# limitz/cuda-audio

Measured on AMD Instinct MI355X. Metric: real-time factor (frames/s / 44.1k), stereo block=256, 10 s IR, higher is better.
Workload: dtype f32

## Files before the change

cuda_audio_amd/csrc/mcconv.hip:

```cpp
#include <hip/hip_runtime.h>
#include <immintrin.h>

#include <algorithm>
#include <atomic>
#include <chrono>
#include <cmath>
#include <cstdarg>
#include <cstdio>
#include <cstdlib>
#include <cstring>
#include <mutex>
#include <new>
#include <vector>

#include "../../include/mcconv.h"
#include "params_handoff.h"
#include "kernels.hip.h"
#include "ossave.hip.h"
#include "singlefft.hip.h"
#include "resample.hip.h"
#include "irshape.hip.h"
#include "ireq.hip.h"
#include "irdecay.hip.h"

// ... 1104 lines not shown
            if (pe[nv] <= pb[nv]) continue;
            list[nv] = act[a];
            if (per_slot_gains) list[nv].uniform = false;
            nv++;
        }
        mo->nsum = std::max(1, nv) * kNchunk;
        if (!nv) HIP_TRY(hipMemsetAsync(e->d_part, 0, sizeof(float4) * (size_t)T * MC_NB * mo->nsum, e->stream));
        for (int a = 0; a < nv; a++) {
            launch_mac_stream(e, list[a], pb[a], pe[a], T, slot0, mo->nsum, a * kNchunk);
            mo->swept = std::max(mo->swept, pe[a] - pb[a]);
        }
        mo->ysrc = e->d_part;
        mo->sk = mo->nsum;
        mo->stt = (int64_t)MC_NB * mo->nsum;
    }
    return MC_OK;
}

Retired make_retired(const mc_engine* e) {
    Retired r;
    r.mac = e->d_res_mac;
    r.fix = e->d_res_fix;
    r.rr = e->rr;
    r.end = (int64_t)e->res_end;
    r.b0 = (int64_t)e->epoch_b0;
    return r;
}

int zero_ring_range(mc_engine* e, float* ring, uint64_t from, uint64_t to) {
    if (to <= from) return MC_OK;
    const uint64_t rr = (uint64_t)e->rr;
    const uint64_t a = from & (rr - 1), n = to - from;
    const uint64_t n1 = std::min(n, rr - a);
    for (int c = 0; c < 2; c++) {
        HIP_TRY(hipMemsetAsync(ring + (size_t)c * rr + a, 0, sizeof(float) * n1, e->stream));
        if (n > n1) HIP_TRY(hipMemsetAsync(ring + (size_t)c * rr, 0, sizeof(float) * (n - n1), e->stream));
    }
    return MC_OK;
}

int retire_epoch(mc_engine* e, uint64_t new_delay, bool force = false) {
    if (new_delay == e->cur_delay && !force) return MC_OK;
    if (e->t_front == e->epoch_b0) {
        e->cur_delay = new_delay;
        return MC_OK;
    }
    if (e->pipe_count) return fail(MC_ERR_STATE, "predelay change / voice merge while a batch awaits mc_finish_batch_device");
    if (e->sliced) return fail(MC_ERR_STATE, "predelay change / voice merge on a block-sliced engine (mc_reset first)");
    {
        int rc = drain_post(e);
        if (!rc) rc = leave_jack_path(e);
        if (rc) return rc;
    }
    const uint64_t b0 = e->t_front, bs = e->epoch_b0, d_old = e->cur_delay;
    const uint64_t new_end = (b0 - (uint64_t)e->pm) * MC_B + e->cfg.n_ref;
    const uint64_t pending_from = std::max<uint64_t>(e->res_end, b0 * MC_B);
    int rc = zero_ring_range(e, e->d_res_mac, pending_from, new_end);
    if (!rc) rc = zero_ring_range(e, e->d_res_fix, pending_from, new_end);
    if (rc) return rc;

    ActiveVoice act[MC_MAXV];
    int vir[2][MC_MAXV];
    const int nact = collect_voices(e, nullptr, act, vir, nullptr);
    int F = 0;
    for (int a = 0; a < nact; a++) F = std::max(F, act[a].p_end);
    F = (int)std::min<uint64_t>((uint64_t)F, (new_end - b0 * MC_B + MC_B - 1) / MC_B);
    if (d_old)
        hipLaunchKernelGGL(k_flush_ring, dim3((unsigned)((d_old + 255) / 256)), dim3(256), 0, e->stream, e->d_wet, e->wr,
                           (int64_t)(b0 * MC_B), (int64_t)d_old, e->d_res_mac, e->rr, (int64_t)new_end);
    uint64_t tv = b0;
    while (F > 0) {
        int Tc = std::min(F, e->Tcap);
        if (!(Tc >= e->stream_threshold && !e->half)) Tc = std::min(Tc, e->Tstream);
        const int slot0 = (int)(tv & (uint64_t)(e->ring - 1));
        hipLaunchKernelGGL(k_fwd<false>, dim3((Tc + FWD_TILE - 1) / FWD_TILE), dim3(XF_THREADS), 0, e->stream, (const float*)nullptr,
                           (const float*)nullptr, 1, (int64_t)0, Tc, e->d_fdl, e->ring, slot0, (const BlockParams*)nullptr, 0,
                           (float4*)nullptr, (float4*)nullptr, e->d_tw, e->d_fdl16, (float*)nullptr, 0, (float4*)nullptr, 0,
                           (int64_t)0, 0, Tc, Tc, 0, 0, DropAhead(), 0);
        MacOut mo;
        rc = launch_mac_batch(e, act, nact, true, Tc, slot0, &mo);
        if (rc) return rc;
        launch_inv(e, mo, tv, e->stream);
        hipLaunchKernelGGL(k_flush_ola, dim3(Tc), dim3(256), 0, e->stream, e->d_seg, e->sr, (int64_t)tv, (int64_t)d_old,
                           e->d_res_mac, e->rr, (int64_t)new_end);
        tv += (uint64_t)Tc;
        F -= Tc;
    }
    {
        const uint64_t n = new_end - b0 * MC_B;
        hipLaunchKernelGGL(k_flush_fix, dim3((unsigned)((n + MC_B - 1) / MC_B)), dim3(256), 0, e->stream, e->d_cring, e->rc,
                           e->d_res_fix, e->rr, (int64_t)(b0 * MC_B), (int64_t)new_end, (int64_t)bs, (int64_t)b0 - 1, (int64_t)d_old,
                           (int64_t)e->cfg.n_ref, (int)e->cfg.compat, make_taildrop(e, vir, d_old), e->pm);
    }
    HIP_TRY(hipGetLastError());
    HIP_TRY(hipMemsetAsync(e->d_fdl, 0, sizeof(float4) * (size_t)MC_NB * e->ring, e->stream));
    if (e->d_fdl16) HIP_TRY(hipMemsetAsync(e->d_fdl16, 0, sizeof(uint2) * (size_t)MC_NB * e->ring, e->stream));
    HIP_TRY(hipMemsetAsync(e->d_seg, 0, sizeof(float) * (size_t)e->sr * 2 * FFT_N, e->stream));
    HIP_TRY(hipMemsetAsync(e->d_wet, 0, sizeof(float) * 2 * (size_t)e->wr, e->stream));
    e->res_end = new_end;
    e->epoch_b0 = b0;
    e->cur_delay = new_delay;
    e->spec_valid = e->dspec.valid = false;
    return MC_OK;
}

void corr_chunks(CorrArgs* ca, int T, int need_a0, int need_a1, int need_b0) {
    ca->need_a0 = need_a0;
    ca->need_a1 = need_a1;
    ca->need_b0 = need_b0;
    ca->run0 = need_a0 & ~(CORR_CHUNK - 1);
    ca->nrun0 = need_a1 > ca->run0 ? (std::min(need_a1, T) - ca->run0 + CORR_CHUNK - 1) / CORR_CHUNK : 0;
    const int end0 = ca->run0 + ca->nrun0 * CORR_CHUNK;
    ca->run1 = std::max(std::min(need_b0, T - 1) & ~(CORR_CHUNK - 1), end0);
    const int nrun1 = T > ca->run1 ? (T - ca->run1 + CORR_CHUNK - 1) / CORR_CHUNK : 0;
    ca->nchunks = ca->nrun0 + nrun1;
}

bool os_applies(const mc_engine* e, const Staged& st, int count, bool slice, const float* d_in1, const float* d_in2, const float* d_outL,
                const float* d_outR, bool q8_ok, int* ovl_blocks) {
    if (!e->os_on || e->os_hold || e->pipelined || (e->sliced && !slice)) return false;
    if (e->cfg.part_begin || e->cfg.part_end || !d_outL || !d_outR || count < e->os_min_blocks || st.ctx.pstride != 0 || st.nact <= 0) return false;
    if (!e->half && count < e->stream_threshold) return false;
    if ((reinterpret_cast<uintptr_t>(d_in1) | reinterpret_cast<uintptr_t>(d_in2) | reinterpret_cast<uintptr_t>(d_outL) | reinterpret_cast<uintptr_t>(d_outR)) & 15) return false;
    int pmax = 0;
    for (int a = 0; a < st.nact; a++) {
        if (!st.act[a].uniform) return false;
        pmax = std::max(pmax, st.act[a].p_end);
    }
    const int ovl = slice ? std::max(pmax, (int)(e->cfg.n_ref / MC_B) + MC_MAX_PREDELAY / MC_B + 2) : pmax;
    if (pmax <= 0 || (int64_t)ovl * MC_B > OS_N / 2) return false;
    if (e->res_end > e->t_front * MC_B) return false;
    if (e->epoch_b0 != 0 && e->epoch_b0 + (uint64_t)pmax > e->t_front) return false;
    if (!q8_ok) return false;
    *ovl_blocks = ovl;
    return true;
}

int ensure_os(mc_engine* e, const Staged& st, int nseg) {
    const size_t seg_el = (size_t)OS_ITEMS * OS_N2;
    const size_t want = (size_t)std::max(nseg, 2);
    if (e->os_T_segs < want) {
        HIP_TRY(hipStreamSynchronize(e->stream));
        if (e->d_os_T) (void)hipFree(e->d_os_T);
        e->d_os_T = nullptr;
        e->os_T_segs = 0;
        HIP_TRY(hipMalloc(&e->d_os_T, sizeof(float4) * seg_el * want));
        e->os_T_segs = want;
    }
    if (e->os_part_segs < (size_t)nseg) {
        HIP_TRY(hipStreamSynchronize(e->stream));
        if (e->d_os_part) (void)hipFree(e->d_os_part);
        e->d_os_part = nullptr;
        e->os_part_segs = 0;
        HIP_TRY(hipMalloc(&e->d_os_part, sizeof(float4) * (size_t)OS_TPS * OS_N1 * (size_t)nseg));
        e->os_part_segs = (size_t)nseg;
    }
    if (!e->os_stream) {
        HIP_TRY(hipStreamCreateWithFlags(&e->os_stream, hipStreamNonBlocking));
        for (int i = 0; i < 3; i++) HIP_TRY(hipEventCreateWithFlags(&e->os_ev[i], hipEventDisableTiming));
    }
    if (!e->d_os_SP) HIP_TRY(hipMalloc(&e->d_os_SP, sizeof(float4) * seg_el * 2));
    if (!e->d_os_SP0) HIP_TRY(hipMalloc(&e->d_os_SP0, sizeof(float4) * 2 * OS_N2));
    mc_engine::OsKey key;
    OsMix mix;
    std::memset(&mix, 0, sizeof(mix));
    key.valid = true;
    key.n = st.nact;
    key.gen = e->ir_gen;
    int64_t lmax = 4;
    for (int a = 0; a < MC_MAXV; a++) {
        key.ir0[a] = key.ir1[a] = -1;
        key.g[a][0] = key.g[a][1] = key.g[a][2] = key.g[a][3] = 0.f;
        if (a >= st.nact) continue;
        const ActiveVoice& av = st.act[a];
        key.ir0[a] = (int)(av.ir0 - e->irs);
        key.ir1[a] = (int)(av.ir1 - e->irs);
        key.g[a][0] = av.ugain.x, key.g[a][1] = av.ugain.y, key.g[a][2] = av.ugain.z, key.g[a][3] = av.ugain.w;
        mix.h0[a] = av.ir0->d_h;
        mix.h1[a] = av.ir1->d_h;
        mix.L0[a] = (int)av.ir0->taps;
        mix.L1[a] = (int)av.ir1->taps;
        mix.g[a] = av.ugain;
        lmax = std::max<int64_t>(lmax, std::max<int64_t>(mix.L0[a], mix.L1[a]));
    }
    mix.n = st.nact;
    const mc_engine::OsKey& k0 = e->os_key;
    if (k0.valid && k0.n == key.n && k0.gen == key.gen && !std::memcmp(k0.ir0, key.ir0, sizeof(key.ir0)) &&
        !std::memcmp(k0.ir1, key.ir1, sizeof(key.ir1)) && !std::memcmp(k0.g, key.g, sizeof(key.g)))
        return MC_OK;
    const int64_t np = (lmax + 3) & ~(int64_t)3;
    if (e->os_planes_n < (size_t)np) {
        HIP_TRY(hipStreamSynchronize(e->stream));
        if (e->d_os_planes) (void)hipFree(e->d_os_planes);
        e->d_os_planes = nullptr;
        e->os_planes_n = 0;
        HIP_TRY(hipMalloc(&e->d_os_planes, sizeof(float) * 4 * (size_t)np));
        e->os_planes_n = (size_t)np;
    }
    e->os_key.valid = false;
    hipLaunchKernelGGL(k_os_ir_mix, dim3((unsigned)((np + 255) / 256)), dim3(256), 0, e->stream, mix, e->d_os_planes, np);
    OsGeo G;
    G.hop = OS_N;
    G.ovl = 0;
    G.n_in = np;
    G.tau0 = 0;
    G.base = 0;
    G.wet_end = np;
    G.seg0 = 0;
    for (int i = 0; i < 2; i++) {
        float4* buf = e->d_os_T + seg_el * i;
        hipLaunchKernelGGL(k_os_cols, dim3(OS_TPS), dim3(OS_THREADS), 0, e->stream, e->d_os_planes + (size_t)np * 2 * i,
                           e->d_os_planes + (size_t)np * (2 * i + 1), (const float*)nullptr, 0, G, buf, (float4*)nullptr, e->d_tw);
        hipLaunchKernelGGL(k_os_rows_fwd, dim3(OS_ITEMS), dim3(G2_THREADS), 0, e->stream, buf);
    }
    hipLaunchKernelGGL(k_os_ir_combine, dim3(OS_ITEMS), dim3(512), 0, e->stream, e->d_os_T, e->d_os_T + seg_el, e->d_os_SP, e->d_os_SP0,
                       0.5f / (float)OS_N);
    HIP_TRY(hipGetLastError());
    e->os_key = key;
    e->n_os[1]++;
    return MC_OK;
}

int run_os(mc_engine* e, const Staged& st, mc_engine::BatchCtx& stored, const float* d_in1, const float* d_in2, float* d_outL, float* d_outR,
           int T, int ovl_blocks, int slot0, bool slice, int first, int count, int halo, const DropAhead* q8_da, int q8_shift) {
    const int w0 = slice ? first - halo : 0, wn = slice ? count + halo : T;
    const int64_t ovl = (int64_t)ovl_blocks * MC_B, hop = (int64_t)OS_N - ovl;
    const int hop_blocks = (int)(hop / MC_B);
    const int nseg = (wn + hop_blocks - 1) / hop_blocks;
    int rc = ensure_os(e, st, nseg);
    if (rc) return rc;
    const BlockParams* d_ptab = st.d_ptab;
    const hipStream_t main = e->stream;
    const hipStream_t side = reinterpret_cast<uintptr_t>(main) > 2 ? e->os_stream : main;
    if (side != main) {
        HIP_TRY(hipEventRecord(e->os_ev[0], main));
        HIP_TRY(hipStreamWaitEvent(side, e->os_ev[0], 0));
    }
    const int hist_from = (int)std::max<int64_t>(0, (int64_t)T - (int64_t)((e->cfg.n_ref + MC_MAX_PREDELAY) / MC_B + 4));
    DropAhead da;
    std::memset(&da, 0, sizeof(da));
    if (!slice) {
        const int reach = std::max(round_up(e->Pcap, 16) + 64, (int)((e->cfg.n_ref + MC_MAX_PREDELAY) / MC_B) + 8);
        const int from = std::max(0, T - reach) & ~(FWD_TILE - 1);
        if (q8_shift >= 0) {
            hipLaunchKernelGGL(k_fwd<true>, dim3((T + FWD_TILE - 1) / FWD_TILE), dim3(XF_THREADS), 0, side, d_in1, d_in2, 1, (int64_t)T * MC_B, T,
                               e->d_fdl, e->ring, slot0, d_ptab, 0, (float4*)nullptr, e->d_slotgain, e->d_tw, e->d_fdl16, e->d_xhist, e->xr, e->d_gring,
                               e->rc, (int64_t)e->t_front, 0, T, T, hist_from, 0, *q8_da, from);
            const TailDrop tdq = make_taildrop(e, st.ctx.vir, st.ctx.predelay);
            const int nd = std::min(T, q8_shift);
            hipLaunchKernelGGL(k_drop_fft, dim3((nd + DF_WAVES - 1) / DF_WAVES), dim3(64 * DF_WAVES), 0, side, tdq, e->d_dropbuf, (int64_t)st.ctx.t0, 0, nd,
                               (int64_t)st.ctx.predelay, (int64_t)e->cfg.n_ref, e->pm, (int64_t)e->epoch_b0);
            (q8_shift < T ? e->n_drop_ahead : e->n_drop_fft)++;
            stored.drop_done = true;
        } else
            hipLaunchKernelGGL(k_fwd<false>, dim3((T - from + FWD_TILE - 1) / FWD_TILE), dim3(XF_THREADS), 0, side, d_in1, d_in2, 1, (int64_t)T * MC_B, T,
                               e->d_fdl, e->ring, slot0, d_ptab, 0, (float4*)nullptr, e->d_slotgain, e->d_tw, e->d_fdl16, e->d_xhist, e->xr, e->d_gring,
                               e->rc, (int64_t)e->t_front, 0, 0, from, hist_from, from, da, 0);
        MacOut mo;
        const uint64_t b = e->t_front + (uint64_t)T - 1;
        e->stream = side;
        rc = launch_mac_batch(e, st.act, st.nact, false, 1, (int)(b & (uint64_t)(e->ring - 1)), &mo);
        if (!rc) launch_inv(e, mo, b, side);
        e->stream = main;
        if (rc) return rc;
    } else if (stored.need_b0 < T) {
        const int from = stored.need_b0 & ~(FWD_TILE - 1);
        hipLaunchKernelGGL(k_fwd<false>, dim3((T - from + FWD_TILE - 1) / FWD_TILE), dim3(XF_THREADS), 0, side, d_in1, d_in2, 1, (int64_t)T * MC_B, T,
                           e->d_fdl, e->ring, slot0, d_ptab, 0, st.d_sums, e->d_slotgain, e->d_tw, e->d_fdl16, e->d_xhist, e->xr, e->d_gring,
                           e->rc, (int64_t)e->t_front, 0, 0, stored.need_b0, hist_from, from, da, 0);
    }
    const int head = slice ? 0 : (int)std::min<uint64_t>((uint64_t)T, (st.ctx.predelay + MC_B - 1) / MC_B);
    OutArgs oa;
    std::memset(&oa, 0, sizeof(oa));
    oa.in1 = d_in1;
    oa.in2 = d_in2;
    oa.outL = d_outL;
    oa.outR = d_outR;
    oa.ptab = d_ptab;
    oa.pstride = 0;
    oa.cring = e->d_cring;
    oa.rc = e->rc;
    oa.tabs0 = (int64_t)st.ctx.t0;
    oa.predelay = (int64_t)st.ctx.predelay;
    oa.n_ref = (int64_t)e->cfg.n_ref;
    oa.b0 = make_retired(e).b0;
    oa.compat = (int)e->cfg.compat;
    oa.pm = e->pm;
    oa.blk0 = 0;
    oa.drop = (!slice && q8_shift >= 0) ? e->d_dropbuf : nullptr;
    if (slice) {
        oa.out_from = first;
        oa.out_end = first + count;
        oa.out_blk0 = first;
        oa.wet_head = 0;
        oa.wet_from = 1 << 30;
    } else {
        oa.out_from = head;
        oa.out_end = T;
        oa.out_blk0 = 0;
        oa.wet_head = head;
        oa.wet_from = std::max(0, T - (MC_MAX_PREDELAY / MC_B + 8));
    }
    OsGeo G;
    G.hop = hop;
    G.ovl = ovl;
    G.n_in = (int64_t)T * MC_B;
    G.tau0 = (int64_t)e->t_front * MC_B;
// ... 2115 lines not shown
```

cuda_audio_amd/csrc/ossave.hip.h:

```cpp
#pragma once

#define OS_N1 FFT_N
#define OS_N2 G2_N
#define OS_N (OS_N1 * OS_N2)
#define OS_LOG2_N2 13
#define OS_TILE 16
#define OS_THREADS (64 * OS_TILE)
#define OS_WSTR 580
#define OS_TPS (OS_N2 / OS_TILE)
#define OS_ITEMS 256
#define OS_ROWT 17

static_assert(OS_N2 == (1 << OS_LOG2_N2), "row length");

struct OsGeo {
    int64_t hop;
    int64_t ovl;
    int64_t n_in;
    int64_t tau0;
    int64_t base;
    int64_t wet_end;
    int seg0;
};

#ifndef OS_XG
#define OS_XG 16
#endif

__device__ __forceinline__ void os_tile_of(int bid, int& segl, int& tile) {
    segl = bid / OS_TPS;
    const int r = bid % OS_TPS;
#if OS_XG > 1
    const int x = r & 7, i = r >> 3;
    const int grp = (i / OS_XG) * 8 + x;
    tile = grp * OS_XG + (i % OS_XG);
#else
    tile = r;
#endif
}

__device__ __forceinline__ v2f os_cis(float x) {
    float sn, cs;
    sincospif(x, &sn, &cs);
    return v2f{cs, sn};
}

template <int SIGN>
__device__ __forceinline__ void os_twiddles(int n2, int lane, v2f (&w)[8]) {
    const float sc = (float)SIGN * 2.0f / (float)OS_N;
    const v2f base = os_cis((float)(n2 * lane) * sc);
    const v2f s1 = os_cis((float)(n2 * 64) * sc);
    const v2f s2 = vx_mul(s1, s1), s3 = vx_mul(s2, s1), s4 = vx_mul(s2, s2);
    w[0] = base;
    w[1] = vx_mul(base, s1);
    w[2] = vx_mul(base, s2);
    w[3] = vx_mul(base, s3);
    w[4] = vx_mul(base, s4);
    w[5] = vx_mul(w[4], s1);
    w[6] = vx_mul(w[4], s2);
    w[7] = vx_mul(w[4], s3);
}

__global__ __launch_bounds__(OS_THREADS) void k_os_cols(const float* __restrict__ in1, const float* __restrict__ in2,
                                                        const float* __restrict__ xhist, int xr, OsGeo G,
                                                        float4* __restrict__ Tbuf, float4* __restrict__ part,
                                                        const float2* __restrict__ g_tw) {
    __shared__ float2 s_tw[FFT_N];
    __shared__ __align__(16) float2 s_mem[OS_TILE * OS_WSTR];
    static_assert(OS_TILE * OS_WSTR >= OS_N1 * OS_ROWT, "staging tile fits");
    static_assert(OS_TILE * OS_WSTR >= OS_ITEMS * OS_ROWT * 2, "transposed tile fits");
    load_twiddles(s_tw, g_tw);
    const int tid = threadIdx.x, lane = tid & 63, wave = tid >> 6;
    int segl, tile;
    os_tile_of((int)blockIdx.x, segl, tile);
    const int n2_0 = tile * OS_TILE;
    const int64_t seg = (int64_t)G.seg0 + segl;
    const int64_t sbase = G.base + seg * G.hop - G.ovl + n2_0;
#pragma unroll
    for (int it = 0; it < 2; it++) {
        const int e = tid + OS_THREADS * it, n1 = e >> 2, q = e & 3;
        const int64_t src = sbase + (int64_t)OS_N2 * n1 + 4 * q;
        float4 a = make_float4(0.f, 0.f, 0.f, 0.f), b = a;
        if (src >= 0) {
            if (src < G.n_in) {
                a = *reinterpret_cast<const float4*>(in1 + src);
                b = *reinterpret_cast<const float4*>(in2 + src);
            }
        } else if (xhist && G.tau0 + src >= 0) {
            const size_t at = (size_t)((G.tau0 + src) & (int64_t)(xr - 1));
            a = *reinterpret_cast<const float4*>(xhist + at);
            b = *reinterpret_cast<const float4*>(xhist + xr + at);
        }
        float2* z = s_mem + n1 * OS_ROWT + 4 * q;
        z[0] = make_float2(a.x, b.x);
        z[1] = make_float2(a.y, b.y);
        z[2] = make_float2(a.z, b.z);
        z[3] = make_float2(a.w, b.w);
        if (part) {
            float s1 = (a.x + a.y) + (a.z + a.w), s2 = (b.x + b.y) + (b.z + b.w);
            float d1 = (a.x - a.y) + (a.z - a.w), d2 = (b.x - b.y) + (b.z - b.w);
            s1 += __shfl_xor(s1, 1), s2 += __shfl_xor(s2, 1), d1 += __shfl_xor(d1, 1), d2 += __shfl_xor(d2, 1);
            s1 += __shfl_xor(s1, 2), s2 += __shfl_xor(s2, 2), d1 += __shfl_xor(d1, 2), d2 += __shfl_xor(d2, 2);
            if (q == 0) part[((size_t)segl * OS_TPS + tile) * OS_N1 + n1] = make_float4(s1, s2, d1, d2);
        }
    }
    __syncthreads();
    float2 v[8];
#pragma unroll
    for (int r = 0; r < 8; r++) v[r] = s_mem[(lane + 64 * r) * OS_ROWT + wave];
    __syncthreads();
    float2* lds = s_mem + wave * OS_WSTR;
    fft512_wave<-1, false>(v, lds, s_tw, lane);
    v2f z[8];
    {
        v2f w[8];
        os_twiddles<-1>(n2_0 + wave, lane, w);
#pragma unroll
        for (int j = 0; j < 8; j++) z[j] = vx_mul(vx_of(lds[lane + 64 * j]), w[j]);
    }
    __syncthreads();
#pragma unroll
    for (int j = 0; j < 8; j++) {
        const int k1 = lane + 64 * j;
        const int item = k1 < 256 ? k1 : ((OS_N1 - k1) & 255), half = k1 >= 256 ? 1 : 0;
        s_mem[(item * OS_ROWT + wave) * 2 + half] = vx_to(z[j]);
    }
    __syncthreads();
    float4* dst = Tbuf + ((size_t)segl * OS_ITEMS << OS_LOG2_N2) + n2_0;
#pragma unroll
    for (int it = 0; it < 4; it++) {
        const int e = tid + OS_THREADS * it, item = e >> 4, c = e & 15;
        dst[((size_t)item << OS_LOG2_N2) + c] = *reinterpret_cast<const float4*>(&s_mem[(item * OS_ROWT + c) * 2]);
    }
}

__device__ __forceinline__ void os_rows0_body(float2* s, const float2* t_lo, const float2* t_hi, float4* __restrict__ row,
                                              const float4* __restrict__ SP0) {
    const int tt = threadIdx.x;
#pragma unroll 1
    for (int c = 0; c < 2; c++) {
        for (int i = tt; i < G2_N; i += G2B_THREADS) s[G2_P(i)] = reinterpret_cast<const float2*>(row + i)[c];
        __syncthreads();
        g2_forward(s, t_lo, t_hi, tt);
        float2 w[G2_N / G2B_THREADS];
#pragma unroll
        for (int m = 0; m < G2_N / G2B_THREADS; m++) {
            const int p = tt + G2B_THREADS * m, pm = c == 0 ? g2_mirror(p) : G2_N - 1 - p;
            const float2 X = s[G2_P(p)], Xm = s[G2_P(pm)];
            const float4 ab = SP0[(size_t)c * G2_N + p];
            w[m] = vx_to(vx_mul(vx_of(X), v2f{ab.x, ab.y}) + vx_mulc(v2f{ab.z, ab.w}, vx_of(Xm)));
        }
        __syncthreads();
#pragma unroll
        for (int m = 0; m < G2_N / G2B_THREADS; m++) s[G2_P(tt + G2B_THREADS * m)] = w[m];
        __syncthreads();
        g2_inverse(s, t_lo, t_hi, tt);
        for (int i = tt; i < G2_N; i += G2B_THREADS) reinterpret_cast<float2*>(row + i)[c] = s[G2_P(i)];
        __syncthreads();
    }
}

__global__ __launch_bounds__(G2B_THREADS, 4) void k_os_rows(float4* __restrict__ Tbuf, const float4* __restrict__ SP,
                                                            const float4* __restrict__ SP0, int nseg) {
    __shared__ float2 s[G2_LDS];
    __shared__ float2 t_lo[128], t_hi[64];
    const int xq = (int)blockIdx.x >> 3;
    const int item = (xq / nseg) * 8 + ((int)blockIdx.x & 7), seg = xq % nseg;
    g2_tables(t_lo, t_hi);
    __syncthreads();
    constexpr int ROWS = G2_N / G2B_THREADS;
    constexpr int PS = 2 * G2B_THREADS + 2 * G2B_THREADS / 32;
    int tt = threadIdx.x;
    asm volatile("" : "+v"(tt));
    float4* row = Tbuf + ((size_t)(seg * OS_ITEMS + item) << OS_LOG2_N2);
    if (item == 0) {
        os_rows0_body(s, t_lo, t_hi, row, SP0);
        return;
    }
    v2f x1[ROWS], x2[ROWS];
    {
        float4 x[ROWS];
#pragma unroll
        for (int r = 0; r < ROWS; r++) x[r] = row[tt + G2B_THREADS * r];
#pragma unroll
        for (int r = 0; r < ROWS; r++) {
            x1[r] = v2f{x[r].x, x[r].y};
            x2[r] = v2f{x[r].z, x[r].w};
        }
    }
    g2_pair<false, 9, false, true>(s, t_lo, t_hi, tt, tt, x1);
    __syncthreads();
    g2_pair<false, 5>(s, t_lo, t_hi, ((tt >> 5) << 9) + (tt & 31), tt & 31);
    G2B_WAVE_SYNC();
    g2_pair<false, 1>(s, t_lo, t_hi, G2B_POS1(tt), (tt >> 5) & 1);
    __syncthreads();
    v2f X1[ROWS];
    {
        asm volatile("" : "+v"(tt));
        const float2* pp = &s[G2_P(2 * tt)];
#pragma unroll
        for (int r = 0; r < ROWS / 2; r++) {
            const v2f a = vx_ld(pp + r * PS), b = vx_ld(pp + r * PS + 1);
            X1[2 * r] = a + b;
            X1[2 * r + 1] = a - b;
        }
    }
    __syncthreads();
    g2_pair<false, 9, false, true>(s, t_lo, t_hi, tt, tt, x2);
    __syncthreads();
    g2_pair<false, 5>(s, t_lo, t_hi, ((tt >> 5) << 9) + (tt & 31), tt & 31);
    G2B_WAVE_SYNC();
    g2_pair<false, 1>(s, t_lo, t_hi, G2B_POS1(tt), (tt >> 5) & 1);
    __syncthreads();
    {
        asm volatile("" : "+v"(tt));
        float2* pm = &s[G2_P(2 * (G2B_THREADS - 1 - tt))];
        constexpr int NP = ROWS / 2, RING = G2B_AHEAD + 1;
        float4 Sq[RING][4];
        const float4* sp = SP + (size_t)item * (NP * 4 * G2B_THREADS) + tt;
        auto request = [&](int r) {
#pragma unroll
            for (int w = 0; w < 4; w++) Sq[r % RING][w] = sp[(size_t)(r * 4 + w) * G2B_THREADS];
        };
#pragma unroll
        for (int r = 0; r < G2B_AHEAD; r++) request(r);
#pragma unroll
        for (int r = 0; r < NP; r++) {
            if (r + G2B_AHEAD < NP) request(r + G2B_AHEAD);
            float2* pb = pm + (NP - 1 - r) * PS;
            const v2f a = vx_ld(pb), b = vx_ld(pb + 1);
            const v2f XB0 = a + b, XB1 = a - b;
            const v2f XA0 = X1[2 * r], XA1 = X1[2 * r + 1];
            const float4 S0 = Sq[r % RING][0], S1 = Sq[r % RING][1], S2 = Sq[r % RING][2], S3 = Sq[r % RING][3];
            const v2f WA0 = vx_mul(XA0, v2f{S0.x, S0.y}) + vx_mulc(v2f{S0.z, S0.w}, XB1);
            const v2f WA1 = vx_mul(XA1, v2f{S1.x, S1.y}) + vx_mulc(v2f{S1.z, S1.w}, XB0);
            const v2f WB1 = vx_mul(XB1, v2f{S2.x, S2.y}) + vx_mulc(v2f{S2.z, S2.w}, XA0);
            const v2f WB0 = vx_mul(XB0, v2f{S3.x, S3.y}) + vx_mulc(v2f{S3.z, S3.w}, XA1);
            vx_st(pb, WB0 + WB1);
            vx_st(pb + 1, WB0 - WB1);
            X1[2 * r] = WA0 + WA1;
            X1[2 * r + 1] = WA0 - WA1;
            __builtin_amdgcn_sched_barrier(0);
        }
    }
    __syncthreads();
    v2f yb[ROWS];
    g2_pair<true, 1>(s, t_lo, t_hi, G2B_POS1(tt), (tt >> 5) & 1);
    G2B_WAVE_SYNC();
    g2_pair<true, 5>(s, t_lo, t_hi, ((tt >> 5) << 9) + (tt & 31), tt & 31);
    __syncthreads();
    g2_pair<true, 9, true, false>(s, t_lo, t_hi, tt, tt, yb);
    __syncthreads();
    {
        asm volatile("" : "+v"(tt));
        float2* pp = &s[G2_P(2 * tt)];
#pragma unroll
        for (int r = 0; r < ROWS / 2; r++) {
            vx_st(pp + r * PS, X1[2 * r]);
            vx_st(pp + r * PS + 1, X1[2 * r + 1]);
        }
    }
    __syncthreads();
    {
        v2f ya[ROWS];
        g2_pair<true, 1>(s, t_lo, t_hi, G2B_POS1(tt), (tt >> 5) & 1);
        G2B_WAVE_SYNC();
        g2_pair<true, 5>(s, t_lo, t_hi, ((tt >> 5) << 9) + (tt & 31), tt & 31);
        __syncthreads();
        g2_pair<true, 9, true, false>(s, t_lo, t_hi, tt, tt, ya);
        asm volatile("" : "+v"(tt));
#pragma unroll
        for (int m = 0; m < ROWS; m++) row[tt + G2B_THREADS * m] = make_float4(ya[m].x, ya[m].y, yb[m].x, yb[m].y);
    }
}

__global__ __launch_bounds__(OS_THREADS) __attribute__((amdgpu_waves_per_eu(8, 8))) void k_os_out(const float4* __restrict__ Tbuf, OsGeo G, float* __restrict__ wet, int wr,
                                                       const float2* __restrict__ g_tw, OutArgs oa) {
    __shared__ float2 s_tw[FFT_N];
    __shared__ __align__(16) float2 s_mem[OS_TILE * OS_WSTR];
    load_twiddles(s_tw, g_tw);
    const int tid = threadIdx.x, lane = tid & 63, wave = tid >> 6;
    int segl, tile;
    os_tile_of((int)blockIdx.x, segl, tile);
    const int n2_0 = tile * OS_TILE;
    const int64_t seg = (int64_t)G.seg0 + segl;
    const float4* src = Tbuf + ((size_t)segl * OS_ITEMS << OS_LOG2_N2) + n2_0;
#pragma unroll
    for (int it = 0; it < 4; it++) {
        const int e = tid + OS_THREADS * it, item = e >> 4, c = e & 15;
        *reinterpret_cast<float4*>(&s_mem[(item * OS_ROWT + c) * 2]) = src[((size_t)item << OS_LOG2_N2) + c];
    }
    __syncthreads();
    float2 v[8];
    {
        v2f w[8];
        os_twiddles<+1>(n2_0 + wave, lane, w);
#pragma unroll
        for (int r = 0; r < 8; r++) {
            const int k1 = lane + 64 * r;
            const int item = k1 < 256 ? k1 : ((OS_N1 - k1) & 255), half = k1 >= 256 ? 1 : 0;
            v[r] = vx_to(vx_mul(vx_of(s_mem[(item * OS_ROWT + wave) * 2 + half]), w[r]));
        }
    }
    __syncthreads();
    fft512_wave<+1, false>(v, s_mem + wave * OS_WSTR, s_tw, lane);
    __syncthreads();
#pragma unroll 1
    for (int it = 0; it < 2; it++) {
        const int e = tid + OS_THREADS * it, n1 = e >> 2, q = e & 3;
        const int64_t n = (int64_t)OS_N2 * n1 + n2_0 + 4 * q;
        const int64_t i0 = G.base + seg * G.hop - G.ovl + n;
        if (n < G.ovl || i0 >= G.wet_end) continue;
        const float2* zz = s_mem + (4 * q) * OS_WSTR + n1;
        const float2 z0 = zz[0], z1 = zz[OS_WSTR], z2 = zz[2 * OS_WSTR], z3 = zz[3 * OS_WSTR];
        const float4 wl4 = make_float4(z0.x, z1.x, z2.x, z3.x), wr4 = make_float4(z0.y, z1.y, z2.y, z3.y);
        const int t = (int)(i0 >> 8);
        if (i0 >= 0 && (t < oa.wet_head || t >= oa.wet_from)) {
            const size_t at = (size_t)((G.tau0 + i0) & (int64_t)(wr - 1));
            *reinterpret_cast<float4*>(wet + at) = wl4;
            *reinterpret_cast<float4*>(wet + wr + at) = wr4;
        }
        const int64_t o0 = i0 + oa.predelay;
        const bool emits = o0 + 3 >= (int64_t)oa.out_from * MC_B && o0 < (int64_t)oa.out_end * MC_B;
        if (!emits) continue;
        const bool whole = ((o0 | oa.n_ref) & 3) == 0 && o0 >= (int64_t)oa.out_from * MC_B;
        const int64_t u0 = oa.tabs0 * MC_B + i0;
        double win[4];
        if (whole) {
            const float4 x1q = *reinterpret_cast<const float4*>(oa.in1 + o0), x2q = *reinterpret_cast<const float4*>(oa.in2 + o0);
            out_window(oa, u0, win);
            const BlockParams& bp = oa.ptab[(o0 >> 8) * oa.pstride];
            float4 d01 = make_float4(0.f, 0.f, 0.f, 0.f), d23 = d01;
            if (oa.drop) {
                const float4* dp = reinterpret_cast<const float4*>(oa.drop + o0);
                d01 = dp[0], d23 = dp[1];
            }
            float4 fl, fr;
            out_frame(false, wl4.x - d01.x, wr4.x - d01.y, x1q.x, x2q.x, bp, win, fl.x, fr.x);
            out_frame(true, wl4.y - d01.z, wr4.y - d01.w, x1q.y, x2q.y, bp, win, fl.y, fr.y);
            out_frame(false, wl4.z - d23.x, wr4.z - d23.y, x1q.z, x2q.z, bp, win, fl.z, fr.z);
            out_frame(true, wl4.w - d23.z, wr4.w - d23.w, x1q.w, x2q.w, bp, win, fl.w, fr.w);
            const int64_t os = o0 - (int64_t)oa.out_blk0 * MC_B;
            *reinterpret_cast<float4*>(oa.outL + os) = fl;
            *reinterpret_cast<float4*>(oa.outR + os) = fr;
        } else {
#pragma unroll 1
            for (int k = 0; k < 4; k++) {
                const int64_t o = o0 + k;
                if (o < (int64_t)oa.out_from * MC_B || o >= (int64_t)oa.out_end * MC_B) continue;
                const BlockParams& bp = oa.ptab[(o >> 8) * oa.pstride];
                const float a = k == 0 ? wl4.x : (k == 1 ? wl4.y : (k == 2 ? wl4.z : wl4.w));
                const float b = k == 0 ? wr4.x : (k == 1 ? wr4.y : (k == 2 ? wr4.z : wr4.w));
                float fl, fr;
                out_window(oa, u0 + k, win);
                const float2 d = oa.drop ? oa.drop[o] : make_float2(0.f, 0.f);
                out_frame((k & 1) != 0, a - d.x, b - d.y, oa.in1[o], oa.in2[o], bp, win, fl, fr);
                oa.outL[o - (int64_t)oa.out_blk0 * MC_B] = fl;
                oa.outR[o - (int64_t)oa.out_blk0 * MC_B] = fr;
            }
        }
    }
}

struct OsMix {
    int n;
    const float2* h0[MC_MAXV];
    const float2* h1[MC_MAXV];
    int L0[MC_MAXV], L1[MC_MAXV];
    float4 g[MC_MAXV];
};

__global__ __launch_bounds__(256) void k_os_ir_mix(OsMix M, float* __restrict__ planes, int64_t np) {
    const int64_t i = (int64_t)blockIdx.x * 256 + threadIdx.x;
    if (i >= np) return;
    float c1r = 0.f, c1i = 0.f, c2r = 0.f, c2i = 0.f;
#pragma unroll
    for (int v = 0; v < MC_MAXV; v++) {
        if (v >= M.n) break;
        if (i < M.L0[v]) {
            const float2 h = M.h0[v][i];
            c1r += M.g[v].x * h.x;
            c1i += M.g[v].z * h.y;
        }
        if (i < M.L1[v]) {
            const float2 h = M.h1[v][i];
            c2r += M.g[v].y * h.x;
            c2i += M.g[v].w * h.y;
        }
    }
    planes[i] = c1r;
    planes[np + i] = c1i;
    planes[2 * np + i] = c2r;
    planes[3 * np + i] = c2i;
}

__global__ __launch_bounds__(G2_THREADS) void k_os_rows_fwd(float4* __restrict__ buf) {
    __shared__ float2 s[2][G2_LDS];
    __shared__ float2 t_lo[128], t_hi[64];
    const int c = threadIdx.x >> 9, tt = threadIdx.x & 511;
    float4* row = buf + ((size_t)blockIdx.x << OS_LOG2_N2);
    g2_tables(t_lo, t_hi);
    for (int i = tt; i < G2_N; i += 512) {
        const float4 v = row[i];
        s[c][G2_P(i)] = c == 0 ? make_float2(v.x, v.y) : make_float2(v.z, v.w);
    }
    __syncthreads();
    g2_forward(s[c], t_lo, t_hi, tt);
    for (int i = threadIdx.x; i < G2_N; i += G2_THREADS) {
        const float2 a = s[0][G2_P(i)], b = s[1][G2_P(i)];
        row[i] = make_float4(a.x, a.y, b.x, b.y);
    }
}

__device__ __forceinline__ float4 os_ab(float2 c1, float2 c2, float sc) {
    return make_float4((c1.x + c2.y) * sc, (c1.y - c2.x) * sc, (c1.x - c2.y) * sc, (c1.y + c2.x) * sc);
}

__global__ __launch_bounds__(512) void k_os_ir_combine(const float4* __restrict__ C1, const float4* __restrict__ C2,
                                                       float4* __restrict__ SP, float4* __restrict__ SP0, float sc) {
    const int item = blockIdx.x, tt = threadIdx.x;
    const float4* r1 = C1 + ((size_t)item << OS_LOG2_N2);
    const float4* r2 = C2 + ((size_t)item << OS_LOG2_N2);
    if (item == 0) {
        for (int p = tt; p < G2_N; p += 512) {
            const float4 a = r1[p], b = r2[p];
            SP0[p] = os_ab(make_float2(a.x, a.y), make_float2(b.x, b.y), sc);
            SP0[G2_N + p] = os_ab(make_float2(a.z, a.w), make_float2(b.z, b.w), sc);
        }
        return;
    }
    float4* sp = SP + (size_t)item * (8 * 4 * 512) + tt;
    for (int r = 0; r < 8; r++) {
        const int j = tt + 512 * r, jp = 4095 - j;
        const float4 a0 = r1[2 * j], a1 = r1[2 * j + 1], b0 = r1[2 * jp], b1 = r1[2 * jp + 1];
        const float4 e0 = r2[2 * j], e1 = r2[2 * j + 1], f0 = r2[2 * jp], f1 = r2[2 * jp + 1];
        sp[(size_t)(r * 4 + 0) * 512] = os_ab(make_float2(a0.x, a0.y), make_float2(e0.x, e0.y), sc);
        sp[(size_t)(r * 4 + 1) * 512] = os_ab(make_float2(a1.x, a1.y), make_float2(e1.x, e1.y), sc);
        sp[(size_t)(r * 4 + 2) * 512] = os_ab(make_float2(b1.z, b1.w), make_float2(f1.z, f1.w), sc);
        sp[(size_t)(r * 4 + 3) * 512] = os_ab(make_float2(b0.z, b0.w), make_float2(f0.z, f0.w), sc);
    }
}
```

Baseline: 1.438 million.

## Widen overlap-save column tiles to 32 frames with two-pass per-wave FFTs

Doubles the column tile width in the overlap-save column and output kernels, so each 16-wave workgroup handles two columns per wave in sequence. Input rows are staged in two halves so each tile reads whole 128-byte lines, and the output stage likewise writes full lines per row. Partial sums keep their 16-frame granularity through a new OS_PPS stride. This trades more registers per thread (forced 8 waves/EU) and extra barriers for fewer workgroups and better-coalesced global accesses.

```diff
diff --git a/cuda_audio_amd/csrc/mcconv.hip b/cuda_audio_amd/csrc/mcconv.hip
--- a/cuda_audio_amd/csrc/mcconv.hip
+++ b/cuda_audio_amd/csrc/mcconv.hip
@@ -1280,7 +1280,7 @@
         if (e->d_os_part) (void)hipFree(e->d_os_part);
         e->d_os_part = nullptr;
         e->os_part_segs = 0;
-        HIP_TRY(hipMalloc(&e->d_os_part, sizeof(float4) * (size_t)OS_TPS * OS_N1 * (size_t)nseg));
+        HIP_TRY(hipMalloc(&e->d_os_part, sizeof(float4) * (size_t)OS_PPS * OS_N1 * (size_t)nseg));
         e->os_part_segs = (size_t)nseg;
     }
     if (!e->os_stream) {
diff --git a/cuda_audio_amd/csrc/ossave.hip.h b/cuda_audio_amd/csrc/ossave.hip.h
--- a/cuda_audio_amd/csrc/ossave.hip.h
+++ b/cuda_audio_amd/csrc/ossave.hip.h
@@ -4,14 +4,29 @@
 #define OS_N2 G2_N
 #define OS_N (OS_N1 * OS_N2)
 #define OS_LOG2_N2 13
-#define OS_TILE 16
-#define OS_THREADS (64 * OS_TILE)
+#define OS_WAVES 16
+#define OS_TILE (2 * OS_WAVES)
+#define OS_THREADS (64 * OS_WAVES)
 #define OS_WSTR 580
+#define OS_LDS (OS_WAVES * OS_WSTR)
 #define OS_TPS (OS_N2 / OS_TILE)
 #define OS_ITEMS 256
 #define OS_ROWT 17
+#define OS_HALF (OS_N1 / 2)
+#define OS_HSTR (OS_TILE + 1)
+#define OS_PART 16
+#define OS_PPS (OS_N2 / OS_PART)
 
 static_assert(OS_N2 == (1 << OS_LOG2_N2), "row length");
+static_assert(OS_N2 % OS_TILE == 0 && MC_B % OS_TILE == 0, "batch, history and segment boundaries (multiples of 256 frames) never cut a tile's 32-frame piece");
+static_assert(OS_TILE * sizeof(float) == 128, "a tile's piece of a row n1 is one whole line");
+static_assert(OS_TILE == 2 * OS_PART && OS_PART == OS_WAVES, "a tile is two 16-frame halves: one column of each per wave, one partial sum each");
+static_assert(OS_WSTR >= FFT_WAVE_LDS, "wave-private transform buffer");
+static_assert(OS_LDS >= OS_HALF * OS_HSTR, "a half pass's staging / output tile fits");
+static_assert(OS_LDS >= OS_ITEMS * OS_ROWT * 2, "transposed tile fits");
+static_assert((OS_LDS + FFT_N) * sizeof(float2) <= 80 * 1024, "two workgroups per CU");
+static_assert(OS_HALF * (OS_TILE / 4) == 2 * OS_THREADS, "two quads of four frames per thread and half pass");
+static_assert(OS_ITEMS * (OS_TILE / 2) == 4 * OS_THREADS, "four 16-byte entries of a transposed tile per thread");
 
 struct OsGeo {
     int64_t hop;
@@ -26,6 +41,7 @@
 #ifndef OS_XG
 #define OS_XG 16
 #endif
+static_assert(OS_XG == 1 || OS_TPS % (8 * OS_XG) == 0, "whole groups of tiles on every XCD");
 
 __device__ __forceinline__ void os_tile_of(int bid, int& segl, int& tile) {
     segl = bid / OS_TPS;
@@ -37,6 +53,12 @@
 #else
     tile = r;
 #endif
+}
+
+__device__ __forceinline__ int os_tid() {
+    int t = threadIdx.x;
+    asm volatile("" : "+v"(t));
+    return t;
 }
 
 __device__ __forceinline__ v2f os_cis(float x) {
@@ -61,14 +83,12 @@
     w[7] = vx_mul(w[4], s3);
 }
 
-__global__ __launch_bounds__(OS_THREADS) void k_os_cols(const float* __restrict__ in1, const float* __restrict__ in2,
+__global__ __launch_bounds__(OS_THREADS) __attribute__((amdgpu_waves_per_eu(8, 8))) void k_os_cols(const float* __restrict__ in1, const float* __restrict__ in2,
                                                         const float* __restrict__ xhist, int xr, OsGeo G,
                                                         float4* __restrict__ Tbuf, float4* __restrict__ part,
                                                         const float2* __restrict__ g_tw) {
     __shared__ float2 s_tw[FFT_N];
-    __shared__ __align__(16) float2 s_mem[OS_TILE * OS_WSTR];
-    static_assert(OS_TILE * OS_WSTR >= OS_N1 * OS_ROWT, "staging tile fits");
-    static_assert(OS_TILE * OS_WSTR >= OS_ITEMS * OS_ROWT * 2, "transposed tile fits");
+    __shared__ __align__(16) float2 s_mem[OS_LDS];
     load_twiddles(s_tw, g_tw);
     const int tid = threadIdx.x, lane = tid & 63, wave = tid >> 6;
     int segl, tile;
@@ -76,61 +96,84 @@
     const int n2_0 = tile * OS_TILE;
     const int64_t seg = (int64_t)G.seg0 + segl;
     const int64_t sbase = G.base + seg * G.hop - G.ovl + n2_0;
-#pragma unroll
-    for (int it = 0; it < 2; it++) {
-        const int e = tid + OS_THREADS * it, n1 = e >> 2, q = e & 3;
-        const int64_t src = sbase + (int64_t)OS_N2 * n1 + 4 * q;
-        float4 a = make_float4(0.f, 0.f, 0.f, 0.f), b = a;
-        if (src >= 0) {
-            if (src < G.n_in) {
-                a = *reinterpret_cast<const float4*>(in1 + src);
-                b = *reinterpret_cast<const float4*>(in2 + src);
+    float2 v[2][8];
+#pragma unroll
+    for (int h = 0; h < 2; h++) {
+        float4 a[2], b[2];
+#pragma unroll
+        for (int it = 0; it < 2; it++) {
+            const int e = tid + OS_THREADS * it, n1 = OS_HALF * h + (e >> 3), q = e & 7;
+            const int64_t src = sbase + (int64_t)OS_N2 * n1 + 4 * q;
+            a[it] = make_float4(0.f, 0.f, 0.f, 0.f), b[it] = a[it];
+            if (src >= 0) {
+                if (src < G.n_in) {
+                    a[it] = *reinterpret_cast<const float4*>(in1 + src);
+                    b[it] = *reinterpret_cast<const float4*>(in2 + src);
+                }
+            } else if (xhist && G.tau0 + src >= 0) {
+                const size_t at = (size_t)((G.tau0 + src) & (int64_t)(xr - 1));
+                a[it] = *reinterpret_cast<const float4*>(xhist + at);
+                b[it] = *reinterpret_cast<const float4*>(xhist + xr + at);
             }
-        } else if (xhist && G.tau0 + src >= 0) {
-            const size_t at = (size_t)((G.tau0 + src) & (int64_t)(xr - 1));
-            a = *reinterpret_cast<const float4*>(xhist + at);
-            b = *reinterpret_cast<const float4*>(xhist + xr + at);
-        }
-        float2* z = s_mem + n1 * OS_ROWT + 4 * q;
-        z[0] = make_float2(a.x, b.x);
-        z[1] = make_float2(a.y, b.y);
-        z[2] = make_float2(a.z, b.z);
-        z[3] = make_float2(a.w, b.w);
-        if (part) {
-            float s1 = (a.x + a.y) + (a.z + a.w), s2 = (b.x + b.y) + (b.z + b.w);
-            float d1 = (a.x - a.y) + (a.z - a.w), d2 = (b.x - b.y) + (b.z - b.w);
-            s1 += __shfl_xor(s1, 1), s2 += __shfl_xor(s2, 1), d1 += __shfl_xor(d1, 1), d2 += __shfl_xor(d2, 1);
-            s1 += __shfl_xor(s1, 2), s2 += __shfl_xor(s2, 2), d1 += __shfl_xor(d1, 2), d2 += __shfl_xor(d2, 2);
-            if (q == 0) part[((size_t)segl * OS_TPS + tile) * OS_N1 + n1] = make_float4(s1, s2, d1, d2);
-        }
-    }
-    __syncthreads();
-    float2 v[8];
-#pragma unroll
-    for (int r = 0; r < 8; r++) v[r] = s_mem[(lane + 64 * r) * OS_ROWT + wave];
-    __syncthreads();
-    float2* lds = s_mem + wave * OS_WSTR;
-    fft512_wave<-1, false>(v, lds, s_tw, lane);
-    v2f z[8];
-    {
-        v2f w[8];
-        os_twiddles<-1>(n2_0 + wave, lane, w);
-#pragma unroll
-        for (int j = 0; j < 8; j++) z[j] = vx_mul(vx_of(lds[lane + 64 * j]), w[j]);
-    }
-    __syncthreads();
-#pragma unroll
-    for (int j = 0; j < 8; j++) {
-        const int k1 = lane + 64 * j;
-        const int item = k1 < 256 ? k1 : ((OS_N1 - k1) & 255), half = k1 >= 256 ? 1 : 0;
-        s_mem[(item * OS_ROWT + wave) * 2 + half] = vx_to(z[j]);
-    }
-    __syncthreads();
+        }
+#pragma unroll
+        for (int it = 0; it < 2; it++) {
+            const int e = tid + OS_THREADS * it, r1 = e >> 3, q = e & 7;
+            const float4 A = a[it], B = b[it];
+            float2* z = s_mem + r1 * OS_HSTR + 4 * q;
+            z[0] = make_float2(A.x, B.x);
+            z[1] = make_float2(A.y, B.y);
+            z[2] = make_float2(A.z, B.z);
+            z[3] = make_float2(A.w, B.w);
+            if (part) {
+                float s1 = (A.x + A.y) + (A.z + A.w), s2 = (B.x + B.y) + (B.z + B.w);
+                float d1 = (A.x - A.y) + (A.z - A.w), d2 = (B.x - B.y) + (B.z - B.w);
+                s1 += __shfl_xor(s1, 1), s2 += __shfl_xor(s2, 1), d1 += __shfl_xor(d1, 1), d2 += __shfl_xor(d2, 1);
+                s1 += __shfl_xor(s1, 2), s2 += __shfl_xor(s2, 2), d1 += __shfl_xor(d1, 2), d2 += __shfl_xor(d2, 2);
+                if ((q & 3) == 0)
+                    part[((size_t)segl * OS_PPS + 2 * tile + (q >> 2)) * OS_N1 + OS_HALF * h + r1] = make_float4(s1, s2, d1, d2);
+            }
+        }
+        __syncthreads();
+#pragma unroll
+        for (int c = 0; c < 2; c++)
+#pragma unroll
+            for (int r = 0; r < 4; r++) v[c][4 * h + r] = s_mem[(lane + 64 * r) * OS_HSTR + wave + OS_WAVES * c];
+        __syncthreads();
+    }
     float4* dst = Tbuf + ((size_t)segl * OS_ITEMS << OS_LOG2_N2) + n2_0;
-#pragma unroll
-    for (int it = 0; it < 4; it++) {
-        const int e = tid + OS_THREADS * it, item = e >> 4, c = e & 15;
-        dst[((size_t)item << OS_LOG2_N2) + c] = *reinterpret_cast<const float4*>(&s_mem[(item * OS_ROWT + c) * 2]);
+#pragma unroll 1
+    for (int c = 0; c < 2; c++) {
+        v2f z[8];
+        {
+            const int t = os_tid(), ln = t & 63;
+            float2* lds = s_mem + (t >> 6) * OS_WSTR;
+            fft512_wave<-1, false>(v[0], lds, s_tw, ln);
+            v2f w[8];
+            os_twiddles<-1>(n2_0 + OS_WAVES * c + (t >> 6), ln, w);
+#pragma unroll
+            for (int j = 0; j < 8; j++) z[j] = vx_mul(vx_of(lds[ln + 64 * j]), w[j]);
+        }
+        __syncthreads();
+        {
+            const int t = os_tid(), ln = t & 63, wv = t >> 6;
+#pragma unroll
+            for (int j = 0; j < 8; j++) {
+                const int k1 = ln + 64 * j;
+                const int item = k1 < 256 ? k1 : ((OS_N1 - k1) & 255), half = k1 >= 256 ? 1 : 0;
+                s_mem[(item * OS_ROWT + wv) * 2 + half] = vx_to(z[j]);
+            }
+        }
+        __syncthreads();
+        const int ts = os_tid();
+#pragma unroll
+        for (int it = 0; it < 4; it++) {
+            const int e = ts + OS_THREADS * it, item = e >> 4, cc = e & 15;
+            dst[((size_t)item << OS_LOG2_N2) + OS_WAVES * c + cc] = *reinterpret_cast<const float4*>(&s_mem[(item * OS_ROWT + cc) * 2]);
+        }
+        __syncthreads();
+#pragma unroll
+        for (int r = 0; r < 8; r++) v[0][r] = v[1][r];
     }
 }
 
@@ -277,88 +320,119 @@
 __global__ __launch_bounds__(OS_THREADS) __attribute__((amdgpu_waves_per_eu(8, 8))) void k_os_out(const float4* __restrict__ Tbuf, OsGeo G, float* __restrict__ wet, int wr,
                                                        const float2* __restrict__ g_tw, OutArgs oa) {
     __shared__ float2 s_tw[FFT_N];
-    __shared__ __align__(16) float2 s_mem[OS_TILE * OS_WSTR];
+    __shared__ __align__(16) float2 s_mem[OS_LDS];
     load_twiddles(s_tw, g_tw);
-    const int tid = threadIdx.x, lane = tid & 63, wave = tid >> 6;
     int segl, tile;
     os_tile_of((int)blockIdx.x, segl, tile);
     const int n2_0 = tile * OS_TILE;
     const int64_t seg = (int64_t)G.seg0 + segl;
     const float4* src = Tbuf + ((size_t)segl * OS_ITEMS << OS_LOG2_N2) + n2_0;
-#pragma unroll
-    for (int it = 0; it < 4; it++) {
-        const int e = tid + OS_THREADS * it, item = e >> 4, c = e & 15;
-        *reinterpret_cast<float4*>(&s_mem[(item * OS_ROWT + c) * 2]) = src[((size_t)item << OS_LOG2_N2) + c];
-    }
-    __syncthreads();
-    float2 v[8];
-    {
-        v2f w[8];
-        os_twiddles<+1>(n2_0 + wave, lane, w);
-#pragma unroll
-        for (int r = 0; r < 8; r++) {
-            const int k1 = lane + 64 * r;
-            const int item = k1 < 256 ? k1 : ((OS_N1 - k1) & 255), half = k1 >= 256 ? 1 : 0;
-            v[r] = vx_to(vx_mul(vx_of(s_mem[(item * OS_ROWT + wave) * 2 + half]), w[r]));
-        }
-    }
-    __syncthreads();
-    fft512_wave<+1, false>(v, s_mem + wave * OS_WSTR, s_tw, lane);
-    __syncthreads();
+    float2 res[2][8];
+#pragma unroll
+    for (int j = 0; j < 8; j++) res[0][j] = make_float2(0.f, 0.f);
 #pragma unroll 1
-    for (int it = 0; it < 2; it++) {
-        const int e = tid + OS_THREADS * it, n1 = e >> 2, q = e & 3;
-        const int64_t n = (int64_t)OS_N2 * n1 + n2_0 + 4 * q;
-        const int64_t i0 = G.base + seg * G.hop - G.ovl + n;
-        if (n < G.ovl || i0 >= G.wet_end) continue;
-        const float2* zz = s_mem + (4 * q) * OS_WSTR + n1;
-        const float2 z0 = zz[0], z1 = zz[OS_WSTR], z2 = zz[2 * OS_WSTR], z3 = zz[3 * OS_WSTR];
-        const float4 wl4 = make_float4(z0.x, z1.x, z2.x, z3.x), wr4 = make_float4(z0.y, z1.y, z2.y, z3.y);
-        const int t = (int)(i0 >> 8);
-        if (i0 >= 0 && (t < oa.wet_head || t >= oa.wet_from)) {
-            const size_t at = (size_t)((G.tau0 + i0) & (int64_t)(wr - 1));
-            *reinterpret_cast<float4*>(wet + at) = wl4;
-            *reinterpret_cast<float4*>(wet + wr + at) = wr4;
-        }
-        const int64_t o0 = i0 + oa.predelay;
-        const bool emits = o0 + 3 >= (int64_t)oa.out_from * MC_B && o0 < (int64_t)oa.out_end * MC_B;
-        if (!emits) continue;
-        const bool whole = ((o0 | oa.n_ref) & 3) == 0 && o0 >= (int64_t)oa.out_from * MC_B;
-        const int64_t u0 = oa.tabs0 * MC_B + i0;
-        double win[4];
-        if (whole) {
-            const float4 x1q = *reinterpret_cast<const float4*>(oa.in1 + o0), x2q = *reinterpret_cast<const float4*>(oa.in2 + o0);
-            out_window(oa, u0, win);
-            const BlockParams& bp = oa.ptab[(o0 >> 8) * oa.pstride];
-            float4 d01 = make_float4(0.f, 0.f, 0.f, 0.f), d23 = d01;
-            if (oa.drop) {
-                const float4* dp = reinterpret_cast<const float4*>(oa.drop + o0);
-                d01 = dp[0], d23 = dp[1];
+    for (int c = 0; c < 2; c++) {
+        const int tl = os_tid();
+#pragma unroll
+        for (int it = 0; it < 4; it++) {
+            const int e = tl + OS_THREADS * it, item = e >> 4, cc = e & 15;
+            *reinterpret_cast<float4*>(&s_mem[(item * OS_ROWT + cc) * 2]) = src[((size_t)item << OS_LOG2_N2) + OS_WAVES * c + cc];
+        }
+        __syncthreads();
+        float2 v[8];
+        {
+            const int t = os_tid(), ln = t & 63, wv = t >> 6;
+            v2f w[8];
+            os_twiddles<+1>(n2_0 + OS_WAVES * c + wv, ln, w);
+#pragma unroll
+            for (int r = 0; r < 8; r++) {
+                const int k1 = ln + 64 * r;
+                const int item = k1 < 256 ? k1 : ((OS_N1 - k1) & 255), half = k1 >= 256 ? 1 : 0;
+                v[r] = vx_to(vx_mul(vx_of(s_mem[(item * OS_ROWT + wv) * 2 + half]), w[r]));
             }
-            float4 fl, fr;
-            out_frame(false, wl4.x - d01.x, wr4.x - d01.y, x1q.x, x2q.x, bp, win, fl.x, fr.x);
-            out_frame(true, wl4.y - d01.z, wr4.y - d01.w, x1q.y, x2q.y, bp, win, fl.y, fr.y);
-            out_frame(false, wl4.z - d23.x, wr4.z - d23.y, x1q.z, x2q.z, bp, win, fl.z, fr.z);
-            out_frame(true, wl4.w - d23.z, wr4.w - d23.w, x1q.w, x2q.w, bp, win, fl.w, fr.w);
-            const int64_t os = o0 - (int64_t)oa.out_blk0 * MC_B;
-            *reinterpret_cast<float4*>(oa.outL + os) = fl;
-            *reinterpret_cast<float4*>(oa.outR + os) = fr;
-        } else {
+        }
+        __syncthreads();
+        {
+            const int t = os_tid(), ln = t & 63;
+            float2* lds = s_mem + (t >> 6) * OS_WSTR;
+            fft512_wave<+1, false>(v, lds, s_tw, ln);
+#pragma unroll
+            for (int j = 0; j < 8; j++) res[1][j] = lds[ln + 64 * j];
+        }
+        if (c == 0) {
+#pragma unroll
+            for (int j = 0; j < 8; j++) res[0][j] = res[1][j];
+        }
+        __syncthreads();
+    }
 #pragma unroll 1
-            for (int k = 0; k < 4; k++) {
-                const int64_t o = o0 + k;
-                if (o < (int64_t)oa.out_from * MC_B || o >= (int64_t)oa.out_end * MC_B) continue;
-                const BlockParams& bp = oa.ptab[(o >> 8) * oa.pstride];
-                const float a = k == 0 ? wl4.x : (k == 1 ? wl4.y : (k == 2 ? wl4.z : wl4.w));
-                const float b = k == 0 ? wr4.x : (k == 1 ? wr4.y : (k == 2 ? wr4.z : wr4.w));
-                float fl, fr;
-                out_window(oa, u0 + k, win);
-                const float2 d = oa.drop ? oa.drop[o] : make_float2(0.f, 0.f);
-                out_frame((k & 1) != 0, a - d.x, b - d.y, oa.in1[o], oa.in2[o], bp, win, fl, fr);
-                oa.outL[o - (int64_t)oa.out_blk0 * MC_B] = fl;
-                oa.outR[o - (int64_t)oa.out_blk0 * MC_B] = fr;
+    for (int h = 0; h < 2; h++) {
+        const int td = os_tid();
+#pragma unroll
+        for (int c = 0; c < 2; c++)
+#pragma unroll
+            for (int j = 0; j < 4; j++) s_mem[((td & 63) + 64 * j) * OS_HSTR + (td >> 6) + OS_WAVES * c] = res[c][j];
+#pragma unroll
+        for (int c = 0; c < 2; c++)
+#pragma unroll
+            for (int j = 0; j < 4; j++) res[c][j] = res[c][4 + j];
+        __syncthreads();
+#pragma unroll 1
+        for (int it = 0; it < 2; it++) {
+            const int e = os_tid() + OS_THREADS * it, r1 = e >> 3, q = e & 7, n1 = OS_HALF * h + r1;
+            const int64_t n = (int64_t)OS_N2 * n1 + n2_0 + 4 * q;
+            const int64_t i0 = G.base + seg * G.hop - G.ovl + n;
+            if (n < G.ovl || i0 >= G.wet_end) continue;
+            const float2* zz = s_mem + r1 * OS_HSTR + 4 * q;
+            const float2 z0 = zz[0], z1 = zz[1], z2 = zz[2], z3 = zz[3];
+            const float4 wl4 = make_float4(z0.x, z1.x, z2.x, z3.x), wr4 = make_float4(z0.y, z1.y, z2.y, z3.y);
+            const int t = (int)(i0 >> 8);
+            if (i0 >= 0 && (t < oa.wet_head || t >= oa.wet_from)) {
+                const size_t at = (size_t)((G.tau0 + i0) & (int64_t)(wr - 1));
+                *reinterpret_cast<float4*>(wet + at) = wl4;
+                *reinterpret_cast<float4*>(wet + wr + at) = wr4;
             }
-        }
+            const int64_t o0 = i0 + oa.predelay;
+            const bool emits = o0 + 3 >= (int64_t)oa.out_from * MC_B && o0 < (int64_t)oa.out_end * MC_B;
+            if (!emits) continue;
+            const bool whole = ((o0 | oa.n_ref) & 3) == 0 && o0 >= (int64_t)oa.out_from * MC_B;
+            const int64_t u0 = oa.tabs0 * MC_B + i0;
+            double win[4];
+            if (whole) {
+                const float4 x1q = *reinterpret_cast<const float4*>(oa.in1 + o0), x2q = *reinterpret_cast<const float4*>(oa.in2 + o0);
+                out_window(oa, u0, win);
+                const BlockParams& bp = oa.ptab[(o0 >> 8) * oa.pstride];
+                float4 d01 = make_float4(0.f, 0.f, 0.f, 0.f), d23 = d01;
+                if (oa.drop) {
+                    const float4* dp = reinterpret_cast<const float4*>(oa.drop + o0);
+                    d01 = dp[0], d23 = dp[1];
+                }
+                float4 fl, fr;
+                out_frame(false, wl4.x - d01.x, wr4.x - d01.y, x1q.x, x2q.x, bp, win, fl.x, fr.x);
+                out_frame(true, wl4.y - d01.z, wr4.y - d01.w, x1q.y, x2q.y, bp, win, fl.y, fr.y);
+                out_frame(false, wl4.z - d23.x, wr4.z - d23.y, x1q.z, x2q.z, bp, win, fl.z, fr.z);
+                out_frame(true, wl4.w - d23.z, wr4.w - d23.w, x1q.w, x2q.w, bp, win, fl.w, fr.w);
+                const int64_t os = o0 - (int64_t)oa.out_blk0 * MC_B;
+                *reinterpret_cast<float4*>(oa.outL + os) = fl;
+                *reinterpret_cast<float4*>(oa.outR + os) = fr;
+            } else {
+#pragma unroll 1
+                for (int k = 0; k < 4; k++) {
+                    const int64_t o = o0 + k;
+                    if (o < (int64_t)oa.out_from * MC_B || o >= (int64_t)oa.out_end * MC_B) continue;
+                    const BlockParams& bp = oa.ptab[(o >> 8) * oa.pstride];
+                    const float a = k == 0 ? wl4.x : (k == 1 ? wl4.y : (k == 2 ? wl4.z : wl4.w));
+                    const float b = k == 0 ? wr4.x : (k == 1 ? wr4.y : (k == 2 ? wr4.z : wr4.w));
+                    float fl, fr;
+                    out_window(oa, u0 + k, win);
+                    const float2 d = oa.drop ? oa.drop[o] : make_float2(0.f, 0.f);
+                    out_frame((k & 1) != 0, a - d.x, b - d.y, oa.in1[o], oa.in2[o], bp, win, fl, fr);
+                    oa.outL[o - (int64_t)oa.out_blk0 * MC_B] = fl;
+                    oa.outR[o - (int64_t)oa.out_blk0 * MC_B] = fr;
+                }
+            }
+        }
+        __syncthreads();
     }
 }
 
```

Result: faster. 1.474 million (median of 6 runs) (+2.5%).
